# jonathandw743/black_hole_ray_marching

Measured on AMD Instinct MI355X. Metric: Mpix/s at 4096×2048, 512 RK steps; max |Δpixel| vs WGSL ref, higher is better.
Workload: dtype f32

## Files before the change

### black_hole_ray_marching_amd/__init__.py

```python
from ._abi import (BH_BLOOM_AUTO, BH_BLOOM_LITERAL, BH_FATE_BLACKOUT, BH_FATE_CAP, BH_FATE_ESCAPE, BH_FATE_SURFACE, BH_LAYOUT_ROWMAJOR,
                   BH_LAYOUT_TILES, BH_LAYOUT_TILES_RGB, BH_LAYOUT_TILES_RGBM, BH_LAYOUT_TILES_RGBM14, BH_UNPACK_RGBM14, BH_ORDER_STATES, BH_BLOOM_SETS, BH_MAX_FRAMES, BH_MATH_EXACT, BH_MATH_FAST, BH_OUT_BGRA8_SRGB, BH_OUT_RGBA16F,
                   BH_OUT_RGBA32F, BH_SCENE_DEFAULT, BH_SCENE_DISC, BH_SCENE_MARKERS, BH_SCHED_FLAG_STATIC_ORDER, BH_SCHED_FLAG_ISSUE_ORDER, BH_SCHED_FLAG_LATENCY, BH_SCHED_PAIR, BH_SCHED_PERSISTENT, BH_SCHED_TILE,
                   BH_LENS_BLACKOUT, BH_LENS_SURFACE, BYTES_PER_PIXEL,
                   BhError, load)
from .scene import (MAX_ITERATIONS, Camera, CameraController, CameraUniform, FrameBatch, Partition, Presenter, Scene, Sky, Uniforms, bloom_check, bloom_plan_failures, clock_mhz, lens_shade_host, load_sky, sky_mips_host,
                    partition_map, refine_cover_host, refine_mask_host, shard_tile_count, shutter_resolve_host, srgb_encode_table, ss_resolve_host, tiles_unpack_rgbm_partition,
                    synthetic_sky, tile_bytes, tiles_unpack, tiles_unpack_rgb, tiles_unpack_rgbm)
from . import raymap

__version__ = "0.5.0"
```

### black_hole_ray_marching_amd/_abi.py

```python
from __future__ import annotations

import ctypes as C
import os
from pathlib import Path

LIB_PATH = Path(os.environ.get("BH_LIB", Path(__file__).resolve().parent / "libbh_render.so"))

BH_OK = 0
BH_ERR_INVALID_ARG = -1
BH_ERR_UNSUPPORTED = -2
BH_ERR_HIP = -3
BH_ERR_NO_DEVICE = -4
BH_ERR_OUT_OF_MEMORY = -5
BH_ERR_INTERNAL = -6

BH_OUT_RGBA32F, BH_OUT_RGBA16F, BH_OUT_BGRA8_SRGB = 0, 1, 2
BH_BLOOM_AUTO, BH_BLOOM_LITERAL = 0, 1
BH_MATH_EXACT, BH_MATH_FAST = 0, 1
BH_SCENE_DISC, BH_SCENE_MARKERS = 1, 2
BH_SCENE_DEFAULT = 3
BH_LAYOUT_ROWMAJOR, BH_LAYOUT_TILES, BH_LAYOUT_TILES_RGB, BH_LAYOUT_TILES_RGBM, BH_LAYOUT_TILES_RGBM14 = 0, 1, 2, 3, 4
BH_UNPACK_RGBM14 = 0x100
BH_ORDER_STATES = 32
BH_BLOOM_SETS = 4
# ... 147 lines not shown
    "bh_tiles_unpack_rgb_rows": (C.c_int, [C.c_void_p, C.c_void_p, C.c_uint32, C.c_uint32, C.c_uint32,
                                           C.c_uint64, C.c_uint32, C.c_uint32, C.c_void_p]),
    "bh_tiles_unpack_rgbm": (C.c_int, [C.c_void_p, C.c_void_p, C.c_void_p, C.c_uint32, C.c_uint32, C.c_uint32,
                                       C.c_uint64, C.c_uint32, C.c_uint32, C.c_void_p]),
    "bh_tile_bytes": (C.c_int64, [C.c_uint32, C.c_uint32]),
    "bh_partition_create": (C.c_int, [C.c_uint32, C.c_uint32, C.c_uint32, C.POINTER(C.c_uint32), C.c_int,
                                      C.POINTER(C.c_void_p)]),
    "bh_partition_destroy": (C.c_int, [C.c_void_p]),
    "bh_partition_tile_count": (C.c_int64, [C.c_void_p, C.c_uint32]),
    "bh_partition_map": (C.c_int, [C.c_uint32, C.c_uint32, C.c_uint32, C.POINTER(C.c_uint32), C.c_void_p,
                                   C.c_void_p]),
    "bh_tiles_unpack_rgbm_partition": (C.c_int, [C.c_void_p, C.c_void_p, C.c_void_p, C.c_void_p, C.c_uint64,
                                                 C.c_uint32, C.c_uint32, C.c_void_p]),
    "bh_srgb_encode_table": (C.c_int, [C.c_void_p]),
    "bh_div_magic_misses": (C.c_int64, [C.c_uint32, C.c_uint32, C.POINTER(C.c_uint32)]),
    "bh_controller_update": (C.c_int, [C.POINTER(bh_controller), C.POINTER(bh_camera), C.c_float, C.c_int,
                                       C.POINTER(C.c_int)]),
    "bh_bloom": (C.c_int, [C.c_void_p, C.c_void_p, C.c_void_p, C.c_uint32, C.c_uint32, C.c_uint32, C.c_uint32,
                           C.c_void_p, C.c_void_p]),
    "bh_bloom_check": (C.c_int, [C.c_uint32, C.c_uint32, C.c_uint32, C.c_uint32, C.POINTER(C.c_uint64), C.c_char_p,
                                 C.c_size_t]),
    "bh_presenter_create": (C.c_int, [C.c_void_p, C.POINTER(bh_presenter_desc), C.POINTER(C.c_void_p)]),
    "bh_presenter_destroy": (C.c_int, [C.c_void_p]),
    "bh_present_frames": (C.c_int, [C.c_void_p, C.c_uint32, C.POINTER(bh_camera_uniform), C.POINTER(bh_uniforms),
                                    C.POINTER(C.c_void_p), C.c_void_p]),
    "bh_present": (C.c_int, [C.c_void_p, C.POINTER(bh_camera_uniform), C.POINTER(bh_uniforms), C.c_void_p, C.c_void_p]),
    "bh_bloom_plan_failures": (C.c_int64, [C.c_char_p, C.c_size_t]),
    "bh_selftest_crmath": (C.c_int, [C.c_int, C.c_uint64, C.c_uint64, C.POINTER(C.c_uint64), C.c_void_p, C.c_int]),
    "bh_set_clock_probe": (C.c_int, [C.c_void_p, C.c_void_p, C.c_uint32]),
    "bh_graph_release": (C.c_int, [C.c_void_p]),
# ... 43 lines not shown
```

### black_hole_ray_marching_amd/csrc/bh_common.hpp

```cpp
#pragma once
#include <hip/hip_runtime.h>
#include <stddef.h>
#include <stdint.h>

#include <string>

#include "../../include/bh_render.h"

namespace bh {

template <uint32_t V>
struct Const { static constexpr uint32_t value = V; };
template <class F>
__attribute__((visibility("hidden"))) inline int with_format(uint32_t format, F&& f) {
    switch (format) {
        case BH_OUT_RGBA32F: return f(Const<BH_OUT_RGBA32F>{});
        case BH_OUT_RGBA16F: return f(Const<BH_OUT_RGBA16F>{});
        default: return f(Const<BH_OUT_BGRA8_SRGB>{});
    }
}

constexpr uint32_t BH_INLINE_FRAMES = 32;
static_assert(BH_INLINE_FRAMES <= BH_MAX_FRAMES, "inline frames");

struct FrameArgs {
    float pos[3];
    float c0[3], c1[3], c2[3];
    float cps[3];
    void* out_col;
    void* out_blackout;
    uint16_t* dbg_n_rk;
    uint8_t* dbg_fate;
    uint16_t* dbg_steps;
};

struct MarchArgs {
    float pos[3];
    float c0[3], c1[3], c2[3];
    float rs, dtm, max_dist, dp;
    uint32_t blackout_eh;
    uint32_t skip_sdf;
    float far_r2;
    uint32_t ss_log2;
    uint32_t ss_out_width;
    uint32_t lens;
    uint32_t width, height, max_iters, scene_flags;
    uint32_t format, layout;
    uint32_t shard_index, shard_count;
    uint32_t tiles_x, tiles_y;
// ... 11 lines not shown
    const float* srgb_lut;
    const float* srgb_enc;
    uint32_t sky_w, sky_h;
    void* out_col;
    void* out_blackout;
    uint16_t* dbg_n_rk;
    uint8_t* dbg_fate;
    uint16_t* dbg_steps;
    uint32_t n_frames;
    uint32_t nf_magic;
    const FrameArgs* frame_table;
    unsigned long long* clk;
    uint32_t clk_mask;
    uint32_t tx_magic;
    FrameArgs frames[BH_INLINE_FRAMES];
};
inline uint32_t div_magic(uint32_t d, uint32_t n_max) {
    if (d < 2u) return 0u;
    const uint64_t m = (1ull << 32) / d + 1u, e = m * d - (1ull << 32);
    return (uint64_t)n_max * e < (1ull << 32) ? (uint32_t)m : 0u;
}
static_assert(sizeof(MarchArgs) + 8 <= 4096, "MarchArgs must fit the kernel argument segment");
static_assert(offsetof(MarchArgs, far_r2) == 72 && offsetof(MarchArgs, ss_log2) == 76 &&
                  offsetof(MarchArgs, ss_out_width) == 80 && offsetof(MarchArgs, lens) == 84 &&
                  offsetof(MarchArgs, width) == 88,
              "MarchArgs: the supersampling words must stay inside the former reserved_[3]");
static_assert(offsetof(MarchArgs, order) == 144 && offsetof(MarchArgs, sky) == 200 && offsetof(MarchArgs, out_col) == 232 &&
                  offsetof(MarchArgs, n_frames) == 272 && offsetof(MarchArgs, frames) == 304 &&
                  sizeof(FrameArgs) == 104 && sizeof(MarchArgs) == 304 + BH_INLINE_FRAMES * sizeof(FrameArgs),
              "MarchArgs: kernel argument layout changed");

struct RefineArgs {
    uint32_t* list;
    uint32_t* ctr;
    const uint8_t* tile_cost;
    uint8_t* mask;
    uint32_t* refined;
    uint32_t width, height;
    uint32_t tiles_x, tiles_y;
    uint32_t n_frames;
    uint32_t capacity;
    uint32_t n_heads;
    float thr;
};

struct LensShadeArgs {
    const bh_lens_px* lens;
    const uint32_t* sky;
    const float* srgb_lut;
    const float* srgb_enc;
    void* out_col;
    void* out_blackout;
    uint32_t width, height;
    uint32_t sky_w, sky_h;
};

struct LensMipArgs : LensShadeArgs {
    const void* chain;
    uint32_t n_levels;
// ... 115 lines not shown
```

### black_hole_ray_marching_amd/csrc/bh_host.cpp

```cpp
#include <hip/hip_runtime.h>

#include <algorithm>
#include <cmath>
#include <cstdlib>
#include <cstring>
#include <limits>
#include <new>
#include <string>
#include <vector>

#include "bh_host.hpp"
#include "bh_srgb.hpp"
#include "bh_lens.hpp"
#include "bh_refine.hpp"
#include "bh_shutter.hpp"
#include "bh_ss.hpp"

namespace {
thread_local std::string g_last_error;
}
static void free_frame_table(bh_ctx::FrameTable& t);

void srgb_lut(float lut[256]) {
    for (int i = 0; i < 256; ++i) {
// ... 240 lines not shown
    if (d->schedule & BH_SCHED_FLAG_ISSUE_ORDER) return true;
    if (d->schedule & BH_SCHED_FLAG_LATENCY) return false;
    const uint64_t tiles = (uint64_t)n_tiles * n_frames;
    return tiles * 512ull >= 384ull * (cus ? cus : 256u) * d->max_iters;
}

static void free_frame_table(bh_ctx::FrameTable& t) {
    for (uint32_t k = 0; k < bh_ctx::FRAME_RING; ++k) {
        if (t.done[k]) { (void)hipEventSynchronize(t.done[k]); (void)hipEventDestroy(t.done[k]); }
        if (t.host[k]) (void)hipHostFree(t.host[k]);
    }
    if (t.dev) (void)hipFree(t.dev);
    t = bh_ctx::FrameTable{};
}

static int stage_frame_table(bh_ctx* c, hipStream_t s, const bh::FrameArgs* frames, uint32_t n,
                             const bh::FrameArgs** dev) {
    if (stream_capturing(s)) {
        g_last_error = "bh_render_frames: more than 32 frames per call cannot be captured into a graph";
        return BH_ERR_UNSUPPORTED;
    }
    bh_ctx::FrameTable* t = nullptr;
    for (auto& x : c->frame_tables)
        if (x.stream == (void*)s) t = &x;
    if (!t) {
        bh_ctx::FrameTable n_t;
        n_t.stream = (void*)s;
        const size_t bytes = sizeof(bh::FrameArgs) * BH_MAX_FRAMES;
        hipError_t he = hipMalloc(&n_t.dev, bytes);
        for (uint32_t k = 0; he == hipSuccess && k < bh_ctx::FRAME_RING; ++k) {
            he = hipHostMalloc(&n_t.host[k], bytes, hipHostMallocDefault);
            if (he == hipSuccess) he = hipEventCreateWithFlags(&n_t.done[k], hipEventDisableTiming);
        }
        if (he != hipSuccess) {
            free_frame_table(n_t);
            return alloc_fail(he, "frame table");
        }
        c->frame_tables.push_back(n_t);
        t = &c->frame_tables.back();
    }
    *dev = t->dev;
    if (t->last.size() == n && std::memcmp(t->last.data(), frames, sizeof(bh::FrameArgs) * n) == 0) return BH_OK;
    const uint32_t k = t->next;
    t->next = (k + 1u) % bh_ctx::FRAME_RING;
    hipError_t he = hipEventSynchronize(t->done[k]);
    if (he == hipSuccess) {
        std::memcpy(t->host[k], frames, sizeof(bh::FrameArgs) * n);
        he = hipMemcpyAsync(t->dev, t->host[k], sizeof(bh::FrameArgs) * n, hipMemcpyHostToDevice, s);
    }
    if (he == hipSuccess) he = hipEventRecord(t->done[k], s);
    if (he != hipSuccess) {
        t->last.clear();
        return hip_fail(he, "frame table upload");
    }
    t->last.assign(frames, frames + n);
    return BH_OK;
}

static int order_state(bh_ctx* c, const bh_render_desc* d, uint64_t nt, hipStream_t s, bool capturing,
                       bh_ctx::OrderState** out, bool from_map = false) {
    const uint64_t pser = d->partition ? d->partition->serial : 0u;
    for (auto& o : c->orders)
        if (o.matches(d, pser, nt, s, from_map)) {
            o.last_use = ++c->order_clock;
            if (capturing) {
                if (!o.valid) {
                    g_last_error = "bh_render: this (geometry, shard, stream) must be rendered once outside graph capture";
                    return BH_ERR_UNSUPPORTED;
                }
                o.captured = true;
// ... 37 lines not shown
}

static void frame_args(const bh_camera_uniform* cam, float rs, const bh_render_desc* d, bh::FrameArgs* F) {
    for (int k = 0; k < 3; ++k) {
        F->pos[k] = cam->pos[k];
        F->c0[k] = cam->world_tri[0][k];
        F->c1[k] = cam->world_tri[1][k];
        F->c2[k] = cam->world_tri[2][k];
    }
    const float x = F->pos[0], y = F->pos[1], z = F->pos[2];
    const float len = std::sqrt((x * x + y * y) + z * z);
    const float n[3] = {x / len, y / len, z / len};
    for (int k = 0; k < 3; ++k) F->cps[k] = (-n[k] * 1.5f) * rs;
    F->out_col = d->out_col; F->out_blackout = d->out_blackout;
    F->dbg_n_rk = d->dbg_n_rk; F->dbg_fate = d->dbg_fate; F->dbg_steps = d->dbg_steps;
}

static uint64_t frame_cost_key(const bh_camera_uniform* cam, const bh_uniforms* U, const bh_render_desc* d,
                               const float* ray_map = nullptr, const bh_ray_pose* poses = nullptr, uint32_t n_poses = 0u,
                               const float* origin_map = nullptr) {
    uint64_t h = 1469598103934665603ull;
    auto mix = [&](const void* p, size_t n) {
        const unsigned char* b = static_cast<const unsigned char*>(p);
        for (size_t i = 0; i < n; ++i) h = (h ^ b[i]) * 1099511628211ull;
    };
    mix(cam->pos, sizeof(float) * 3);
    for (int k = 0; k < 3; ++k) mix(cam->world_tri[k], sizeof(float) * 3);
    for (int k = 0; k < 3; ++k) mix(cam->screen_tri[k], sizeof(float) * 3);
    mix(&U->rs, 4); mix(&U->delta_time_mult, 4); mix(&U->blackout_eh, 4); mix(&U->max_dist, 4);
    mix(&U->distortion_power, 4);
// ... 47 lines not shown
        const char* why = e->layout != BH_LAYOUT_ROWMAJOR      ? "a row-major output (BH_LAYOUT_ROWMAJOR)"
                          : e->shard_count != 1u               ? "the whole frame (shard_count 1)"
                          : e->partition                       ? "no partition"
                          : (e->schedule & 0xFFu) != BH_SCHED_TILE ? "the tile schedule (BH_SCHED_TILE)"
                          : (e->dbg_n_rk || e->dbg_fate || e->dbg_steps) ? "no dbg_* outputs (they are per ray, not per pixel)"
                                                               : nullptr;
        if (why) return why;
    }
    return nullptr;
}

struct Launch {
    bh_render_desc d;
    bh::MarchArgs a;
    std::vector<bh::FrameArgs> table;
    uint64_t n_tiles = 0;
    uint32_t shutter_log2 = 0;
    const float* ray_map = nullptr;
    const bh_ray_pose* poses = nullptr;
    const float* origin_map = nullptr;
};

static int check_launch(const bh_ctx* c, uint32_t n_frames, const bh_camera_uniform* cams, const bh_uniforms* U,
                        const bh_render_desc* descs, uint32_t ss, Launch* L) {
    if (!c || !cams || !U || !descs || n_frames == 0 || n_frames > BH_MAX_FRAMES) return bad_arg(__func__, __LINE__);
    const bh_render_desc* const d0 = &descs[0];
    L->d = *d0;
    if (ss > 1u) { L->d.width *= ss; L->d.height *= ss; }
    const bh_render_desc* d = &L->d;
    if (!d->out_col) return bad_arg(__func__, __LINE__);
// ... 54 lines not shown
    a.order_block = (uint32_t)((L->n_tiles + a.tiles_y - 1u) / a.tiles_y);
    a.order_centre = bh_tile_row(&cams[0], d->height);
    a.sky = c->sky; a.srgb_lut = c->lut; a.srgb_enc = c->enc; a.sky_w = c->sky_w; a.sky_h = c->sky_h;
    a.kfac = (a.dp * a.rs) * -1.5f;
    a.rw2 = 1.0f / (2.0f * (float)a.width);
    a.rh2 = 1.0f / (2.0f * (float)a.height);
    a.n_frames = n_frames;
    const uint64_t slots = L->n_tiles * n_frames;
    a.nf_magic = slots - 1u <= 0xFFFFFFFFull ? bh::div_magic(n_frames, (uint32_t)(slots - 1u)) : 0u;
    a.tx_magic = a.shard_count == 1u && a.n_tiles != 0u ? bh::div_magic(a.tiles_x, a.n_tiles - 1u) : 0u;
    a.clk = c->clk;
    a.clk_mask = c->clk_mask;
    if (n_frames > bh::BH_INLINE_FRAMES) L->table.resize(n_frames);
    bh::FrameArgs* fa = L->table.empty() ? a.frames : L->table.data();
    for (uint32_t i = 0; i < n_frames; ++i) frame_args(&cams[i], a.rs, &descs[i], &fa[i]);
    const bh::FrameArgs& F = fa[0];
    for (int k = 0; k < 3; ++k) {
        a.pos[k] = F.pos[k]; a.c0[k] = F.c0[k]; a.c1[k] = F.c1[k]; a.c2[k] = F.c2[k]; a.cps[k] = F.cps[k];
    }
    a.out_col = F.out_col; a.out_blackout = F.out_blackout;
    a.dbg_n_rk = F.dbg_n_rk; a.dbg_fate = F.dbg_fate; a.dbg_steps = F.dbg_steps;
}

static int stage_frames(bh_ctx* c, hipStream_t s, Launch* L) {
    if (L->table.empty()) return BH_OK;
    return stage_frame_table(c, s, L->table.data(), L->a.n_frames, &L->a.frame_table);
}

static int learned_order(bh_ctx* c, Launch* L, const bh_camera_uniform* cam0, const bh_uniforms* U, hipStream_t s,
                         bh_ctx::OrderState** out) {
    const bh_render_desc* d = &L->d;
    bh::MarchArgs& a = L->a;
    *out = nullptr;
    if ((d->schedule & 0xFFu) != BH_SCHED_TILE || (d->schedule & BH_SCHED_FLAG_STATIC_ORDER)) return BH_OK;
    bh_ctx::OrderState* os = nullptr;
    int st = order_state(c, d, L->n_tiles, s, stream_capturing(s), &os, L->ray_map != nullptr);
    if (st != BH_OK) return st;
    if (!os->valid) {
        hipError_t he = hipMemsetAsync(os->counters, 0, bh::ORDER_WORDS * sizeof(uint32_t), s);
        if (he == hipSuccess) he = hipMemsetAsync(os->tile_cost, 0, L->n_tiles, s);
        if (he != hipSuccess) return hip_fail(he, "temporal order reset");
// ... 540 lines not shown
```

### black_hole_ray_marching_amd/csrc/bh_host.hpp

```cpp
#pragma once
#include <hip/hip_runtime.h>

#include <array>
#include <cstring>
#include <memory>
#include <string>
#include <vector>

#include "bh_common.hpp"
#include "bh_srgb.hpp"

#define BH_HIDDEN __attribute__((visibility("hidden")))
#define BH_INTERNAL extern "C" BH_HIDDEN

struct bh_ctx {
    int device = 0;
    uint32_t* sky = nullptr;
    float* lut = nullptr;
    float* enc = nullptr;
    uint8_t* enc_b = nullptr;
    uint32_t* enc_e = nullptr;
    uint32_t* counters = nullptr;
    uint32_t sky_w = 0, sky_h = 0;
    uint32_t grid_exact = 0, grid_fast = 0;
// ... 24 lines not shown
        void free_buffers() {
            (void)hipFree(tile_cost); (void)hipFree(order); (void)hipFree(counters);
            (void)hipFree(refine_list); (void)hipFree(refine_ctr); (void)hipFree(refine_mask);
        }
    };
    std::vector<OrderState> orders;
    uint64_t order_clock = 0;
    static constexpr uint32_t FRAME_RING = 4;
    struct FrameTable {
        void* stream = nullptr;
        bh::FrameArgs* dev = nullptr;
        bh::FrameArgs* host[FRAME_RING] = {};
        hipEvent_t done[FRAME_RING] = {};
        uint32_t next = 0;
        std::vector<bh::FrameArgs> last;
    };
    std::vector<FrameTable> frame_tables;
    struct SepPlan {
        std::array<uint32_t, 6> key{};
        uint32_t* dev = nullptr;
        int ext = 0;
        uint32_t nc = 0, nr = 0;
        size_t rec = 0;
        size_t stc = 0;
        uint32_t stw = 0;
        uint32_t* strips = nullptr;
        std::shared_ptr<std::vector<uint32_t>> host;
    };
    struct BloomScratch {
        uint64_t key = 0;
// ... 137 lines not shown
```

### black_hole_ray_marching_amd/csrc/bh_march_ray.hpp

```cpp
#pragma once
#include "bh_march_step.hpp"

namespace bh {
namespace BH_NS {

constexpr uint32_t PRIO_ITERS = 48;

constexpr uint32_t WG_WAVES = 1u;

struct Hist { v3 ro, rd; float tr; uint32_t outside; };

__device__ __forceinline__ bool same_bits(float x, float y) { return __float_as_uint(x) == __float_as_uint(y); }
__device__ __forceinline__ bool same_state(const RayState& st, const Hist& h) {
    return same_bits(st.ro.x, h.ro.x) & same_bits(st.ro.y, h.ro.y) & same_bits(st.ro.z, h.ro.z) &
           same_bits(st.rd.x, h.rd.x) & same_bits(st.rd.y, h.rd.y) & same_bits(st.rd.z, h.rd.z) &
           same_bits(st.travelled, h.tr) & (st.outside == h.outside);
}

struct HistLds { float4 a[2][2][64]; };
__device__ __forceinline__ uint32_t state_hash(const RayState& st) {
    return (__float_as_uint(st.ro.x) ^ __float_as_uint(st.ro.y) ^ __float_as_uint(st.ro.z) ^
            __float_as_uint(st.rd.x) ^ __float_as_uint(st.rd.y) ^ __float_as_uint(st.rd.z) ^
            __float_as_uint(st.travelled)) + st.outside * 0x9E3779B9u;
}
// ... 35 lines not shown
                    const float4 r0 = H.a[p][0][lane], r1 = H.a[p][1][lane];
                    st.ro = mk(r0.x, r0.y, r0.z); st.rd = mk(r1.x, r1.y, r1.z); st.travelled = r0.w;
                }
                st.n_rk = a.max_iters;
                return BH_FATE_CAP;
            }
        }
        h2 = h1;
    }
    for (;;) {
        const uint32_t fate = march_step_tail<SF>(a, f, st);
        if (fate != 0xFFu) { steps = st.n_rk; return fate; }
    }
}

template <uint32_t SF, bool SHUT = false>
__device__ __forceinline__ void march_ray(const MarchArgs& a, const Frame& f, RayState& st, uint32_t& fate,
                                          uint32_t& steps, uint32_t lane) {
    RayState sb = st;
    bool alive = true;
    constexpr uint32_t TRIP_PAIRS = 3;
    static_assert(PRIO_ITERS % (2u * TRIP_PAIRS) == 0u, "whole trips");
    for (uint32_t it = 0; it < PRIO_ITERS && __builtin_amdgcn_ballot_w64(alive) != 0ull; it += 2u * TRIP_PAIRS) {
#pragma unroll
        for (uint32_t j = 0; j < TRIP_PAIRS; ++j) {
            if (alive) {
                if (march_step_io<SF, true>(a, f, st, sb, fate, it + 2u * j)) {
                    alive = false;
                    if (fate_before_rk(fate)) sb.n_rk = 0u;
                }
            }
            if (alive) {
                if (march_step_io<SF, true>(a, f, sb, st, fate, it + 2u * j + 1u)) {
                    alive = false;
                    if (fate_before_rk(fate)) st.n_rk = 0u;
                }
            }
        }
// ... 12 lines not shown
```

### black_hole_ray_marching_amd/csrc/bh_march_step.hpp

```cpp
#pragma once
#include "bh_march_ops.hpp"

namespace bh {
namespace BH_NS {


struct Frame {
    v3 ro0;
    v3 cps;
    float k;
};
__device__ __forceinline__ Frame make_frame(const MarchArgs& a) {
    Frame f;
    f.ro0 = mk(a.pos[0], a.pos[1], a.pos[2]);
    f.cps = mk(a.cps[0], a.cps[1], a.cps[2]);
    f.k = a.kfac;
    return f;
}

__device__ __forceinline__ v3 pixel_ray(const MarchArgs& a, uint32_t px, uint32_t py) {
#if BH_FAST
    const float l0 = ((float)px + 0.5f) / (2.0f * (float)a.width);
    const float l2 = ((float)py + 0.5f) / (2.0f * (float)a.height);
#else
// ... 352 lines not shown
    G.bad |= !(G.amin >= crm::ACC_N_MIN);
    if constexpr (!CO) G.bad |= !(fabsf(s) <= 0x1p30f);
    const float ntr = travelled + dt;
    out.s = s;
    out.outside = CO ? 1u : (not_out ? in.outside : 1u);
    out.ro = unpk(padd(ro, dro));
    out.rd = unpk(padd(rd, drd));
    out.travelled = ntr;
    out.n_rk = n_rk + 1u;
    const bool escape = ntr > a.max_dist;
    fate = escape ? (uint32_t)BH_FATE_ESCAPE : (uint32_t)BH_FATE_CAP;
    return escape | (n_rk + 1u >= a.max_iters);
}
#endif

template <uint32_t SF = SF_DYN, bool UNI = false, bool TINY = false>
__device__ __forceinline__ bool march_step_io(const MarchArgs& a, const Frame& f, const RayState& in, RayState& out,
                                              uint32_t& fate, uint32_t it = 0u) {
#if BH_FAST
    FOps X;
    return step_bf<true, FOps, SF, UNI>(a, f, in, out, X, fate, it);
#else
    XOps<true> X;
#ifdef BH_DIAG_SLOW
    if ((threadIdx.x & 63u) == (uint32_t)__builtin_ctzll(__builtin_amdgcn_ballot_w64(true)))
        atomicAdd(&g_diag_all_wave_steps, 1u);
#endif
    bool done = step_bf<true, XOps<true>, SF, UNI, TINY>(a, f, in, out, X, fate, it);
#ifdef BH_DIAG_SLOW
    const uint64_t badm = __builtin_amdgcn_ballot_w64(X.bad);
// ... 75 lines not shown
```

### black_hole_ray_marching_amd/csrc/bh_march_tile.hpp

```cpp
#pragma once
#include "bh_march_ray.hpp"
#include "bh_march_resolve.hpp"
#include "bh_march_shade.hpp"
#include "bh_refine.hpp"

namespace bh {
namespace BH_NS {


#define BH_CONST_AS __attribute__((address_space(4)))
template <class T>
__device__ __forceinline__ const BH_CONST_AS T* const_as(const T* p) { return (const BH_CONST_AS T*)p; }
__device__ __forceinline__ const BH_CONST_AS FrameArgs* frame_args_of(const MarchArgs& A, uint32_t fi) {
    return (A.frame_table ? const_as(A.frame_table) : const_as(&A.frames[0])) + fi;
}
struct FrameCamera { float pos[3], c0[3], c1[3], c2[3], cps[3]; };
__device__ __forceinline__ FrameCamera load_camera(const BH_CONST_AS FrameArgs* F) {
    FrameCamera c;
    for (int k = 0; k < 3; ++k) {
        c.pos[k] = F->pos[k]; c.c0[k] = F->c0[k]; c.c1[k] = F->c1[k]; c.c2[k] = F->c2[k]; c.cps[k] = F->cps[k];
    }
    return c;
}
__device__ __forceinline__ void select_camera(MarchArgs& a, const FrameCamera& c) {
    for (int k = 0; k < 3; ++k) {
        a.pos[k] = c.pos[k]; a.c0[k] = c.c0[k]; a.c1[k] = c.c1[k]; a.c2[k] = c.c2[k]; a.cps[k] = c.cps[k];
    }
}
__device__ __forceinline__ void select_outputs(MarchArgs& a, const BH_CONST_AS FrameArgs* F) {
    a.out_col = F->out_col; a.out_blackout = F->out_blackout;
    a.dbg_n_rk = F->dbg_n_rk; a.dbg_fate = F->dbg_fate; a.dbg_steps = F->dbg_steps;
}

struct SlotHead {
    uint32_t fi, t, tx, ty;
    FrameCamera cam;
    bool ok;
};
template <bool ITEM>
__device__ __forceinline__ SlotHead slot_head(const MarchArgs& A, uint32_t slot, uint32_t item_tx = 0u, uint32_t item_ty = 0u) {
    SlotHead h{};
    const uint32_t nf = A.n_frames;
    uint32_t fi = 0, j = slot;
    if constexpr (ITEM) {
        fi = slot;
    } else if (nf > 1u) {
        j = A.nf_magic ? __umulhi(slot, A.nf_magic) : slot / nf;
        fi = slot - j * nf;
    }
    h.fi = fi;
    h.cam = load_camera(frame_args_of(A, fi));
    if constexpr (ITEM) {
        h.tx = item_tx;
        h.ty = item_ty;
    } else {
        const uint32_t t = A.order ? const_as(A.order)[j] : centre_out(j, A.n_tiles, A.order_block, A.order_centre);
        h.t = t;
        if (t >= A.n_tiles) return h;
        if (A.tile_list) {
            const uint32_t v = const_as(A.tile_list)[t];
            h.tx = v & 0xFFFFu;
            h.ty = v >> 16;
        } else if (A.shard_count == 1u && A.tx_magic) {
            h.ty = __umulhi(t, A.tx_magic);
            h.tx = t - h.ty * A.tiles_x;
        } else {
            shard_tile_coords(t, A.tiles_x, A.shard_index, A.shard_count, &h.tx, &h.ty);
        }
    }
    h.ok = true;
    return h;
}

constexpr uint32_t F_SS = 1u, F_ITEM = 2u, F_LENS = 4u, F_SHUT = 8u, F_RAYS = 16u, F_POSE = 32u, F_ORG = 64u;
struct ShutterLane { uint32_t px, py; bool valid, ok; };
struct OrgRay { v3 d, ro0; };
__device__ __forceinline__ OrgRay org_load(const MarchArgs& a, const float* dirs, const float* orgs, uint32_t px,
                                           uint32_t py, bool valid) {
    OrgRay g;
    g.d = mk(0.0f, 0.0f, 1.0f);
    g.ro0 = mk(a.pos[0], a.pos[1], a.pos[2]);
    if (valid) {
        const size_t i = ((size_t)py * a.width + px) * 3u;
        const float* p = dirs + i;
        const float* q = orgs + i;
        const v3 m = mk(p[0], p[1], p[2]);
        const v3 o = mk(q[0], q[1], q[2]);
        const v3 r = mk(a.c0[0], a.c0[1], a.c0[2]), u = mk(a.c1[0], a.c1[1], a.c1[2]), fw = mk(a.c2[0], a.c2[1], a.c2[2]);
        g.d = add(add(smul(m.x, r), smul(m.y, u)), smul(m.z, fw));
// ... 56 lines not shown
            const float* p = dirs + ((size_t)py * a.width + px) * 3u;
            d = mk(p[0], p[1], p[2]);
            if constexpr (POSE)
                d = add(add(smul(d.x, mk(a.c0[0], a.c0[1], a.c0[2])), smul(d.y, mk(a.c1[0], a.c1[1], a.c1[2]))),
                        smul(d.z, mk(a.c2[0], a.c2[1], a.c2[2])));
        }
        st.rd = normalize_x(d);
    } else
#endif
    st.rd = pixel_ray(a, valid ? px : 0u, valid ? py : 0u);
    st.s = ray_s(f, st.rd);
    st.travelled = 0.0f;
    st.n_rk = 0;
    st.outside = 0u;
    uint32_t fate = 0xFFu, steps = 0;
    if (valid) {
        if constexpr (SF != SF_DYN) {
            const bool out = ORG ? __builtin_amdgcn_ballot_w64(!((dot(f.ro0, f.ro0) > 1.01f) & (fabsf(st.s) <= 0x1p30f))) == 0ull
                                 : (dot(f.ro0, f.ro0) > 1.01f) && (__builtin_amdgcn_ballot_w64(!(fabsf(st.s) <= 0x1p30f)) == 0ull);
            if (__builtin_amdgcn_readfirstlane((int)out)) march_ray<SF | SF_CAM_OUT, SHUT>(a, f, st, fate, steps, lane);
            else march_ray<SF, SHUT>(a, f, st, fate, steps, lane);
        } else {
            march_ray<SF, SHUT>(a, f, st, fate, steps, lane);
        }
    }
    if constexpr (SHUT) {
        shutter_stage(a, lut, lane, valid, fate, st, steps);
        *sl = ShutterLane{px, py, valid, true};
    } else
    if constexpr (SS) {
        uint32_t fo = fi;
        asm volatile("" : "+s"(fo));
        select_outputs(a, frame_args_of(A, fo));
        v3 sc, sb;
        ss_samples(a, lut, lane, valid, fate, st, steps, sc, sb);
        ss_resolve_store<FMT>(a, lut, lane, px, py, valid, sc, sb);
    } else
    if (valid) {
// ... 13 lines not shown
    if (a.tile_cost) {
        const uint32_t m = min(wave_max_u32(steps) >> 1, 255u);
        if (lane == 0u) {
            a.tile_cost[t] = (uint8_t)m;
            const uint32_t b = cost_bucket(m);
            if (b < ORDER_BUCKETS - 1u)
                __hip_atomic_fetch_add(&a.order_tot[b], 1u, __ATOMIC_RELAXED, __HIP_MEMORY_SCOPE_AGENT);
        }
    }
}
template <uint32_t FMT, uint32_t SF, uint32_t FORM>
__device__ __forceinline__ void march_slot(const MarchArgs& A, uint32_t slot, const float* lut,
                                           uint32_t lane, uint32_t item_tx = 0u, uint32_t item_ty = 0u,
                                           ShutterLane* sl = nullptr, const float* dirs = nullptr,
                                           const float* orgs = nullptr) {
    const SlotHead h = slot_head<(FORM & F_ITEM) != 0u>(A, slot, item_tx, item_ty);
    if (!h.ok) return;
    march_slot_body<FMT, SF, FORM>(A, h, lut, lane, sl, dirs, orgs);
}

struct ClockStart { uint32_t t, r; };
__device__ __forceinline__ ClockStart clock_start() {
    return {(uint32_t)__builtin_amdgcn_s_memtime(), (uint32_t)__builtin_amdgcn_s_memrealtime()};
}
__device__ __forceinline__ void clock_end(unsigned long long* acc, const ClockStart& c0) {
    const uint32_t t = (uint32_t)__builtin_amdgcn_s_memtime() - c0.t;
    const uint32_t r = (uint32_t)__builtin_amdgcn_s_memrealtime() - c0.r;
    const uint32_t x = __builtin_amdgcn_s_getreg((3 << 11) | (0 << 6) | 20) & 7u;
    const bool sane = (uint64_t)t >= 5ull * r && (uint64_t)t <= 40ull * r;
    if ((threadIdx.x & 63u) == 0u && sane) {
        unsigned long long* p = acc + 16u * x;
// ... 4 lines not shown
}

template <uint32_t FMT, uint32_t SF, uint32_t FORM>
__device__ __forceinline__ void march_tile_wave(const MarchArgs& A, float* lut, const float* dirs = nullptr,
                                                const float* orgs = nullptr) {
    static_assert(WG_WAVES == 1u, "the table copy is one wave's: 64 lanes x 16 bytes per table");
    static_assert(!(FORM & (F_ITEM | F_SHUT)), "work items and shutter waves have kernels of their own");
    constexpr bool LENS = FORM & F_LENS;
    asm volatile("" ::"s"(A.srgb_lut), "s"(A.n_tiles), "s"(A.n_frames), "s"(A.nf_magic), "s"(A.frame_table),
                 "s"(A.order), "s"(A.tile_list), "s"(A.shard_count), "s"(A.tx_magic), "s"(A.tiles_x), "s"(A.clk),
                 "s"(A.clk_mask), "s"(A.width), "s"(A.height), "s"(A.rw2), "s"(A.rh2));
    SrgbRows<FMT> rows;
    if constexpr (!LENS) rows = srgb_fetch<FMT>(A);
    const uint32_t slot = __builtin_amdgcn_readfirstlane(blockIdx.x * WG_WAVES + (threadIdx.x >> 6));
    if (slot >= A.n_tiles * A.n_frames) return;
    const SlotHead h = slot_head<false>(A, slot);
    if constexpr (!LENS) {
        srgb_store<FMT>(rows, lut);
        __syncthreads();
    }
    const bool probe = A.clk && ((slot + (slot >> 8)) & A.clk_mask) == 0u;
    ClockStart c0{0u, 0u};
    if (probe) c0 = clock_start();
    if (h.ok) march_slot_body<FMT, SF, FORM>(A, h, lut, threadIdx.x & 63u, nullptr, dirs, orgs);
    if (probe) clock_end(A.clk, c0);
}

template <uint32_t FMT, uint32_t SF>
__global__ void __launch_bounds__(64 * WG_WAVES) march_tile_kernel(MarchArgs A) {
    __shared__ __attribute__((aligned(16))) float lut[lds_tables<FMT>()];
    march_tile_wave<FMT, SF, 0u>(A, lut);
// ... 160 lines not shown
```

### black_hole_ray_marching_amd/scene.py

```python
from __future__ import annotations

import ctypes as C
from dataclasses import dataclass, field

import numpy as np

from . import _abi
from ._abi import (BH_LAYOUT_ROWMAJOR, BH_LAYOUT_TILES, BH_LAYOUT_TILES_RGB, BH_LAYOUT_TILES_RGBM, BH_LAYOUT_TILES_RGBM14, BH_UNPACK_RGBM14, BH_MATH_EXACT, BH_MATH_FAST, BH_OUT_RGBA16F,
                   BH_OUT_RGBA32F, BH_OUT_BGRA8_SRGB, BH_SCENE_DEFAULT, BYTES_PER_PIXEL, BhError, check, load)

MAX_ITERATIONS = 1000


@dataclass
class Camera:
    pos: tuple = (0.0, 0.0, -20.0)
    dir: tuple = (0.0, 0.0, 1.0)
    up: tuple = (0.0, 1.0, 0.0)
    aspect: float = 1.0
    fovy: float = float(np.float32(np.pi) * np.float32(0.5))
    znear: float = 0.1
    zfar: float = 100.0

    @classmethod
# ... 110 lines not shown
    out = np.empty((height, width, 4), dtype=np.uint8)
    check(load().bh_synthetic_sky(out.ctypes.data, width, height, seed), "bh_synthetic_sky")
    return out


def load_sky(path) -> np.ndarray:
    from PIL import Image
    with Image.open(path) as im:
        return np.ascontiguousarray(np.asarray(im.convert("RGBA"), dtype=np.uint8))


def srgb_encode_table() -> np.ndarray:
    out = np.empty(257, np.float32)
    check(load().bh_srgb_encode_table(out.ctypes.data), "bh_srgb_encode_table")
    return out


def shard_tile_count(width: int, height: int, shard_index: int, shard_count: int) -> int:
    n = load().bh_shard_tile_count(width, height, shard_index, shard_count)
    if n < 0:
        raise BhError(int(n), "bh_shard_tile_count")
    return int(n)


def bloom_check(width: int, height: int, levels: int = 3, schedule: int = 0) -> list[tuple]:
    lib = load()
    n = C.c_uint64()
    buf = C.create_string_buffer(1 << 16)
    check(lib.bh_bloom_check(width, height, levels, schedule, C.byref(n), buf, len(buf)), "bh_bloom_check")
    out = []
# ... 734 lines not shown
```

### include/bh_render.h

```cpp
#ifndef BH_RENDER_H
#define BH_RENDER_H

#include <stddef.h>
#include <stdint.h>

#ifdef __cplusplus
extern "C" {
#endif

#define BH_ABI_VERSION 8

#define BH_ORDER_STATES 32
#define BH_BLOOM_SETS 4

typedef enum {
    BH_OK = 0,
    BH_ERR_INVALID_ARG = -1,
    BH_ERR_UNSUPPORTED = -2,
    BH_ERR_HIP = -3,
    BH_ERR_NO_DEVICE = -4,
    BH_ERR_OUT_OF_MEMORY = -5,
    BH_ERR_INTERNAL = -6
} bh_status;

// ... 257 lines not shown
                        bh_partition** out);
int bh_partition_destroy(bh_partition* partition);
int64_t bh_partition_tile_count(const bh_partition* partition, uint32_t shard_index);
int bh_partition_map(uint32_t width, uint32_t height, uint32_t shard_count, const uint32_t* weights, uint32_t* owner_out,
                     uint32_t* index_out);
int bh_tiles_unpack_rgbm_partition(const void* packed, void* out_col, void* out_blackout, const bh_partition* partition,
                                   uint64_t shard_stride_tiles, uint32_t format, uint32_t rows_in_flight,
                                   void* hip_stream);

int64_t bh_tile_bytes(uint32_t layout, uint32_t format);

int bh_srgb_encode_table(float* out257);

int64_t bh_div_magic_misses(uint32_t d, uint32_t n_max, uint32_t* magic);

int bh_selftest_crmath(int op, uint64_t base, uint64_t count, uint64_t* out_mismatches,
                       uint32_t* out_examples, int device);

int bh_set_clock_probe(bh_ctx* ctx, uint64_t* acc, uint32_t stride);

#ifdef __cplusplus
}
#endif

#endif
```

Baseline: 16720.

## Peel first RK step using host-precomputed per-frame step size and radius terms

All rays in a frame start at the camera position, so the first step's SDF distance, step size and 1/r^5 divisor are identical across pixels. The host now computes these once per frame and passes them in the kernel arguments or frame table, and the tile kernel runs a specialised first RK4 step that skips the SDF evaluation and one divide. The main march loop then resumes at iteration 1. This adds kernel-argument bytes, a validity fallback through a wave ballot, and extra code paths that could raise register pressure.

```diff
diff --git a/black_hole_ray_marching_amd/__init__.py b/black_hole_ray_marching_amd/__init__.py
--- a/black_hole_ray_marching_amd/__init__.py
+++ b/black_hole_ray_marching_amd/__init__.py
@@ -3,7 +3,7 @@
                    BH_OUT_RGBA32F, BH_SCENE_DEFAULT, BH_SCENE_DISC, BH_SCENE_MARKERS, BH_SCHED_FLAG_STATIC_ORDER, BH_SCHED_FLAG_ISSUE_ORDER, BH_SCHED_FLAG_LATENCY, BH_SCHED_PAIR, BH_SCHED_PERSISTENT, BH_SCHED_TILE,
                    BH_LENS_BLACKOUT, BH_LENS_SURFACE, BYTES_PER_PIXEL,
                    BhError, load)
-from .scene import (MAX_ITERATIONS, Camera, CameraController, CameraUniform, FrameBatch, Partition, Presenter, Scene, Sky, Uniforms, bloom_check, bloom_plan_failures, clock_mhz, lens_shade_host, load_sky, sky_mips_host,
+from .scene import (MAX_ITERATIONS, Camera, CameraController, CameraUniform, FrameBatch, Partition, Presenter, Scene, Sky, Uniforms, bloom_check, bloom_plan_failures, clock_mhz, first_step_host, lens_shade_host, load_sky, sky_mips_host,
                     partition_map, refine_cover_host, refine_mask_host, shard_tile_count, shutter_resolve_host, srgb_encode_table, ss_resolve_host, tiles_unpack_rgbm_partition,
                     synthetic_sky, tile_bytes, tiles_unpack, tiles_unpack_rgb, tiles_unpack_rgbm)
 from . import raymap
diff --git a/black_hole_ray_marching_amd/_abi.py b/black_hole_ray_marching_amd/_abi.py
--- a/black_hole_ray_marching_amd/_abi.py
+++ b/black_hole_ray_marching_amd/_abi.py
@@ -185,6 +185,8 @@
                                                  C.c_uint32, C.c_uint32, C.c_void_p]),
     "bh_srgb_encode_table": (C.c_int, [C.c_void_p]),
     "bh_div_magic_misses": (C.c_int64, [C.c_uint32, C.c_uint32, C.POINTER(C.c_uint32)]),
+    "bh_first_step_host": (C.c_int, [C.POINTER(bh_camera_uniform), C.POINTER(bh_uniforms), C.c_uint32, C.c_uint32,
+                                     C.POINTER(C.c_float), C.POINTER(C.c_float), C.POINTER(C.c_float)]),
     "bh_controller_update": (C.c_int, [C.POINTER(bh_controller), C.POINTER(bh_camera), C.c_float, C.c_int,
                                        C.POINTER(C.c_int)]),
     "bh_bloom": (C.c_int, [C.c_void_p, C.c_void_p, C.c_void_p, C.c_uint32, C.c_uint32, C.c_uint32, C.c_uint32,
diff --git a/black_hole_ray_marching_amd/csrc/bh_common.hpp b/black_hole_ray_marching_amd/csrc/bh_common.hpp
--- a/black_hole_ray_marching_amd/csrc/bh_common.hpp
+++ b/black_hole_ray_marching_amd/csrc/bh_common.hpp
@@ -33,6 +33,8 @@
     uint8_t* dbg_fate;
     uint16_t* dbg_steps;
 };
+
+struct FirstStep { float dt0, Q0, rq0; };
 
 struct MarchArgs {
     float pos[3];
@@ -74,20 +76,22 @@
     uint32_t clk_mask;
     uint32_t tx_magic;
     FrameArgs frames[BH_INLINE_FRAMES];
+    FirstStep first[BH_INLINE_FRAMES];
 };
 inline uint32_t div_magic(uint32_t d, uint32_t n_max) {
     if (d < 2u) return 0u;
     const uint64_t m = (1ull << 32) / d + 1u, e = m * d - (1ull << 32);
     return (uint64_t)n_max * e < (1ull << 32) ? (uint32_t)m : 0u;
 }
-static_assert(sizeof(MarchArgs) + 8 <= 4096, "MarchArgs must fit the kernel argument segment");
+static_assert(sizeof(MarchArgs) + 16 <= 4096, "MarchArgs must fit the kernel argument segment");
 static_assert(offsetof(MarchArgs, far_r2) == 72 && offsetof(MarchArgs, ss_log2) == 76 &&
                   offsetof(MarchArgs, ss_out_width) == 80 && offsetof(MarchArgs, lens) == 84 &&
                   offsetof(MarchArgs, width) == 88,
               "MarchArgs: the supersampling words must stay inside the former reserved_[3]");
 static_assert(offsetof(MarchArgs, order) == 144 && offsetof(MarchArgs, sky) == 200 && offsetof(MarchArgs, out_col) == 232 &&
                   offsetof(MarchArgs, n_frames) == 272 && offsetof(MarchArgs, frames) == 304 &&
-                  sizeof(FrameArgs) == 104 && sizeof(MarchArgs) == 304 + BH_INLINE_FRAMES * sizeof(FrameArgs),
+                  sizeof(FrameArgs) == 104 && offsetof(MarchArgs, first) == 304 + BH_INLINE_FRAMES * sizeof(FrameArgs) &&
+                  sizeof(FirstStep) == 12 && sizeof(MarchArgs) == 304 + BH_INLINE_FRAMES * (sizeof(FrameArgs) + sizeof(FirstStep)),
               "MarchArgs: kernel argument layout changed");
 
 struct RefineArgs {
@@ -103,6 +107,7 @@
     uint32_t n_heads;
     float thr;
 };
+static_assert(sizeof(MarchArgs) + sizeof(RefineArgs) <= 4096, "march_refine_kernel's arguments must fit the kernel argument segment");
 
 struct LensShadeArgs {
     const bh_lens_px* lens;
diff --git a/black_hole_ray_marching_amd/csrc/bh_host.cpp b/black_hole_ray_marching_amd/csrc/bh_host.cpp
--- a/black_hole_ray_marching_amd/csrc/bh_host.cpp
+++ b/black_hole_ray_marching_amd/csrc/bh_host.cpp
@@ -278,8 +278,8 @@
     t = bh_ctx::FrameTable{};
 }
 
-static int stage_frame_table(bh_ctx* c, hipStream_t s, const bh::FrameArgs* frames, uint32_t n,
-                             const bh::FrameArgs** dev) {
+static int stage_frame_table(bh_ctx* c, hipStream_t s, const bh::FrameArgs* frames, const bh::FirstStep* first,
+                             uint32_t n, const bh::FrameArgs** dev) {
     if (stream_capturing(s)) {
         g_last_error = "bh_render_frames: more than 32 frames per call cannot be captured into a graph";
         return BH_ERR_UNSUPPORTED;
@@ -290,7 +290,7 @@
     if (!t) {
         bh_ctx::FrameTable n_t;
         n_t.stream = (void*)s;
-        const size_t bytes = sizeof(bh::FrameArgs) * BH_MAX_FRAMES;
+        const size_t bytes = (sizeof(bh::FrameArgs) + sizeof(bh::FirstStep)) * BH_MAX_FRAMES;
         hipError_t he = hipMalloc(&n_t.dev, bytes);
         for (uint32_t k = 0; he == hipSuccess && k < bh_ctx::FRAME_RING; ++k) {
             he = hipHostMalloc(&n_t.host[k], bytes, hipHostMallocDefault);
@@ -304,13 +304,17 @@
         t = &c->frame_tables.back();
     }
     *dev = t->dev;
-    if (t->last.size() == n && std::memcmp(t->last.data(), frames, sizeof(bh::FrameArgs) * n) == 0) return BH_OK;
+    const size_t fb = sizeof(bh::FrameArgs) * n, rb = sizeof(bh::FirstStep) * n;
+    if (t->last.size() == n && std::memcmp(t->last.data(), frames, fb) == 0 &&
+        std::memcmp(t->last_first.data(), first, rb) == 0)
+        return BH_OK;
     const uint32_t k = t->next;
     t->next = (k + 1u) % bh_ctx::FRAME_RING;
     hipError_t he = hipEventSynchronize(t->done[k]);
     if (he == hipSuccess) {
-        std::memcpy(t->host[k], frames, sizeof(bh::FrameArgs) * n);
-        he = hipMemcpyAsync(t->dev, t->host[k], sizeof(bh::FrameArgs) * n, hipMemcpyHostToDevice, s);
+        std::memcpy(t->host[k], frames, fb);
+        std::memcpy(reinterpret_cast<unsigned char*>(t->host[k]) + fb, first, rb);
+        he = hipMemcpyAsync(t->dev, t->host[k], fb + rb, hipMemcpyHostToDevice, s);
     }
     if (he == hipSuccess) he = hipEventRecord(t->done[k], s);
     if (he != hipSuccess) {
@@ -318,6 +322,7 @@
         return hip_fail(he, "frame table upload");
     }
     t->last.assign(frames, frames + n);
+    t->last_first.assign(first, first + n);
     return BH_OK;
 }
 
@@ -385,6 +390,60 @@
     for (int k = 0; k < 3; ++k) F->cps[k] = (-n[k] * 1.5f) * rs;
     F->out_col = d->out_col; F->out_blackout = d->out_blackout;
     F->dbg_n_rk = d->dbg_n_rk; F->dbg_fate = d->dbg_fate; F->dbg_steps = d->dbg_steps;
+}
+
+static bool first_step_disabled() {
+    static const bool off = std::getenv("BH_NO_FIRST_STEP") != nullptr;
+    return off;
+}
+
+static bool first_step_record(const float pos[3], const float cps[3], float rs, float dtm, float max_dist,
+                              uint32_t scene_flags, uint32_t max_iters, bh::FirstStep* out) {
+    *out = bh::FirstStep{0.0f, 0.0f, 0.0f};
+    const float x = pos[0], y = pos[1], z = pos[2];
+    const float in[8] = {x, y, z, cps[0], cps[1], cps[2], rs, dtm};
+    for (float v : in)
+        if (!std::isfinite(v)) return false;
+    if (!(dtm > 0.0f) || !(rs > 0.0f) || !(max_iters >= 2u)) return false;
+    const float r2 = (x * x + y * y) + z * z;
+    if (!(r2 > 1.01f && r2 <= 0x1p24f)) return false;
+    const float r0 = std::sqrt(r2);
+    const float dtr = dtm * r0;
+    const float rho = std::sqrt(x * x + z * z);
+    const float disc = std::fmax(std::fmax(rho - 6.0f * rs, -(rho - 3.0f * rs)), std::fabs(y - 0.0f) - 0.02f);
+    const float xx = x * x, yy = y * y;
+    const float dz = -10.0f - z, zz = dz * dz;
+    const float ty = 10.0f - std::fabs(y), tx = 10.0f - std::fabs(x);
+    const float qy = (xx + ty * ty) + zz, qx = (tx * tx + yy) + zz;
+    const float m = std::sqrt(std::fmin(qy, qx)) - 0.5f;
+    float ds;
+    if (!(scene_flags & BH_SCENE_MARKERS)) ds = (scene_flags & BH_SCENE_DISC) ? disc : INFINITY;
+    else ds = (scene_flags & BH_SCENE_DISC) ? std::fmin(disc, m) : m;
+    if (!(ds >= 0.001f)) return false;
+    const float dx = cps[0] - x, dy = cps[1] - y, dzp = cps[2] - z;
+    const float dps = std::sqrt((dx * dx + dy * dy) + dzp * dzp) - 0.075f;
+    const float dist = std::fmin(ds, dps);
+    const float dt0 = std::fmin(dist * 0.9f, dtr);
+    if (!(dt0 >= 0x1p-25f && dt0 <= 0x1p13f) || !(dt0 <= max_dist)) return false;
+    const float Q0 = (r2 * r2) * r0;
+    const float rq0 = 1.0f / Q0;
+    if (!(Q0 >= 0x1p-40f && Q0 <= 0x1p60f)) return false;
+    *out = bh::FirstStep{dt0, Q0, rq0};
+    return true;
+}
+
+int bh_first_step_host(const bh_camera_uniform* cam, const bh_uniforms* U, uint32_t scene_flags, uint32_t max_iters,
+                       float* dt0, float* Q0, float* rq0) {
+    if (!cam || !U) return 0;
+    bh::FrameArgs F;
+    bh_render_desc d{};
+    frame_args(cam, U->rs, &d, &F);
+    bh::FirstStep fs;
+    const bool ok = first_step_record(F.pos, F.cps, U->rs, U->delta_time_mult, U->max_dist, scene_flags, max_iters, &fs);
+    if (dt0) *dt0 = fs.dt0;
+    if (Q0) *Q0 = fs.Q0;
+    if (rq0) *rq0 = fs.rq0;
+    return ok ? 1 : 0;
 }
 
 static uint64_t frame_cost_key(const bh_camera_uniform* cam, const bh_uniforms* U, const bh_render_desc* d,
@@ -462,6 +521,7 @@
     bh_render_desc d;
     bh::MarchArgs a;
     std::vector<bh::FrameArgs> table;
+    std::vector<bh::FirstStep> first_table;
     uint64_t n_tiles = 0;
     uint32_t shutter_log2 = 0;
     const float* ray_map = nullptr;
@@ -546,6 +606,11 @@
     if (n_frames > bh::BH_INLINE_FRAMES) L->table.resize(n_frames);
     bh::FrameArgs* fa = L->table.empty() ? a.frames : L->table.data();
     for (uint32_t i = 0; i < n_frames; ++i) frame_args(&cams[i], a.rs, &descs[i], &fa[i]);
+    if (!L->table.empty()) L->first_table.assign(n_frames, bh::FirstStep{0.0f, 0.0f, 0.0f});
+    bh::FirstStep* fs = L->table.empty() ? a.first : L->first_table.data();
+    if (d->math == BH_MATH_EXACT && (d->schedule & 0xFFu) == BH_SCHED_TILE && !first_step_disabled())
+        for (uint32_t i = 0; i < n_frames; ++i)
+            (void)first_step_record(fa[i].pos, fa[i].cps, a.rs, a.dtm, a.max_dist, a.scene_flags, a.max_iters, &fs[i]);
     const bh::FrameArgs& F = fa[0];
     for (int k = 0; k < 3; ++k) {
         a.pos[k] = F.pos[k]; a.c0[k] = F.c0[k]; a.c1[k] = F.c1[k]; a.c2[k] = F.c2[k]; a.cps[k] = F.cps[k];
@@ -556,7 +621,7 @@
 
 static int stage_frames(bh_ctx* c, hipStream_t s, Launch* L) {
     if (L->table.empty()) return BH_OK;
-    return stage_frame_table(c, s, L->table.data(), L->a.n_frames, &L->a.frame_table);
+    return stage_frame_table(c, s, L->table.data(), L->first_table.data(), L->a.n_frames, &L->a.frame_table);
 }
 
 static int learned_order(bh_ctx* c, Launch* L, const bh_camera_uniform* cam0, const bh_uniforms* U, hipStream_t s,
diff --git a/black_hole_ray_marching_amd/csrc/bh_host.hpp b/black_hole_ray_marching_amd/csrc/bh_host.hpp
--- a/black_hole_ray_marching_amd/csrc/bh_host.hpp
+++ b/black_hole_ray_marching_amd/csrc/bh_host.hpp
@@ -62,6 +62,7 @@
         hipEvent_t done[FRAME_RING] = {};
         uint32_t next = 0;
         std::vector<bh::FrameArgs> last;
+        std::vector<bh::FirstStep> last_first;
     };
     std::vector<FrameTable> frame_tables;
     struct SepPlan {
diff --git a/black_hole_ray_marching_amd/csrc/bh_march_ray.hpp b/black_hole_ray_marching_amd/csrc/bh_march_ray.hpp
--- a/black_hole_ray_marching_amd/csrc/bh_march_ray.hpp
+++ b/black_hole_ray_marching_amd/csrc/bh_march_ray.hpp
@@ -73,14 +73,17 @@
     }
 }
 
-template <uint32_t SF, bool SHUT = false>
+template <uint32_t SF, bool SHUT = false, bool PEEL = false>
 __device__ __forceinline__ void march_ray(const MarchArgs& a, const Frame& f, RayState& st, uint32_t& fate,
-                                          uint32_t& steps, uint32_t lane) {
+                                          uint32_t& steps, uint32_t lane, [[maybe_unused]] const RayState* prev = nullptr,
+                                          [[maybe_unused]] uint32_t it0 = 0u) {
     RayState sb = st;
+    if constexpr (PEEL) sb = *prev;
+    const uint32_t first = PEEL ? it0 : 0u;
     bool alive = true;
     constexpr uint32_t TRIP_PAIRS = 3;
     static_assert(PRIO_ITERS % (2u * TRIP_PAIRS) == 0u, "whole trips");
-    for (uint32_t it = 0; it < PRIO_ITERS && __builtin_amdgcn_ballot_w64(alive) != 0ull; it += 2u * TRIP_PAIRS) {
+    for (uint32_t it = first; it < PRIO_ITERS + first && __builtin_amdgcn_ballot_w64(alive) != 0ull; it += 2u * TRIP_PAIRS) {
 #pragma unroll
         for (uint32_t j = 0; j < TRIP_PAIRS; ++j) {
             if (alive) {
diff --git a/black_hole_ray_marching_amd/csrc/bh_march_step.hpp b/black_hole_ray_marching_amd/csrc/bh_march_step.hpp
--- a/black_hole_ray_marching_amd/csrc/bh_march_step.hpp
+++ b/black_hole_ray_marching_amd/csrc/bh_march_step.hpp
@@ -390,6 +390,40 @@
 }
 #endif
 
+#if !BH_FAST
+__device__ __forceinline__ bool step_first(const RayState& in, RayState& out, const FirstStep& fs) {
+    XOps<true> X;
+    const v3 ro = in.ro, rd = in.rd;
+    const float s = in.s, dt = fs.dt0;
+    const float nx = s * ro.x, ny = s * ro.y, nz = s * ro.z;
+    X.kmin = crm::kmin3(crm::key(nx), crm::key(ny), crm::key(nz));
+    const crm::Rcp R{fs.Q0, fs.rq0};
+    const v3 ro_k1 = smul(dt, rd);
+    const v3 rd_k1 = smul(dt, mk(crm::div_core(nx, R), crm::div_core(ny, R), crm::div_core(nz, R)));
+    const v3 ro_k2 = smul(dt, X.rd_half(rd, rd_k1));
+    const v3 rd_k2 = smul(dt, X.template accel<2>(X.ro_half(ro, ro_k1), s));
+    const v3 ro_k3 = smul(dt, X.rd_half(rd, rd_k2));
+    const v3 rd_k3 = smul(dt, X.template accel<3>(X.ro_half(ro, ro_k2), s));
+    const v3 ro_k4 = smul(dt, add(rd, rd_k3));
+    const v3 rd_k4 = smul(dt, X.template accel<4>(add(ro, ro_k3), s));
+    const v3 sro = add(X.add2(X.add2(ro_k1, ro_k2), ro_k3), ro_k4);
+    const v3 srd = add(X.add2(X.add2(rd_k1, rd_k2), rd_k3), rd_k4);
+    const v3 dro = X.template div6<0>(sro);
+    const v3 drd = X.template div6<1>(srd);
+    X.bad |= X.kmin < crm::KEY_ACC_MIN;
+    X.bad |= !(X.amin >= crm::ACC_N_MIN);
+    X.bad |= !(X.amin6 >= crm::DIV_N_MIN);
+    X.bad |= !(fabsf(s) <= 0x1p30f);
+    out.ro = add(ro, dro);
+    out.rd = add(rd, drd);
+    out.travelled = in.travelled + dt;
+    out.s = s;
+    out.n_rk = in.n_rk + 1u;
+    out.outside = 1u;
+    return X.bad;
+}
+#endif
+
 template <uint32_t SF = SF_DYN, bool UNI = false, bool TINY = false>
 __device__ __forceinline__ bool march_step_io(const MarchArgs& a, const Frame& f, const RayState& in, RayState& out,
                                               uint32_t& fate, uint32_t it = 0u) {
diff --git a/black_hole_ray_marching_amd/csrc/bh_march_tile.hpp b/black_hole_ray_marching_amd/csrc/bh_march_tile.hpp
--- a/black_hole_ray_marching_amd/csrc/bh_march_tile.hpp
+++ b/black_hole_ray_marching_amd/csrc/bh_march_tile.hpp
@@ -35,9 +35,15 @@
 struct SlotHead {
     uint32_t fi, t, tx, ty;
     FrameCamera cam;
+    FirstStep fs;
     bool ok;
 };
-template <bool ITEM>
+__device__ __forceinline__ FirstStep load_first_step(const MarchArgs& A, uint32_t fi) {
+    const BH_CONST_AS FirstStep* p = A.frame_table ? (const BH_CONST_AS FirstStep*)(const_as(A.frame_table) + A.n_frames)
+                                                   : const_as(&A.first[0]);
+    return {p[fi].dt0, p[fi].Q0, p[fi].rq0};
+}
+template <bool ITEM, bool FS = false>
 __device__ __forceinline__ SlotHead slot_head(const MarchArgs& A, uint32_t slot, uint32_t item_tx = 0u, uint32_t item_ty = 0u) {
     SlotHead h{};
     const uint32_t nf = A.n_frames;
@@ -50,6 +56,7 @@
     }
     h.fi = fi;
     h.cam = load_camera(frame_args_of(A, fi));
+    if constexpr (FS) h.fs = load_first_step(A, fi);
     if constexpr (ITEM) {
         h.tx = item_tx;
         h.ty = item_ty;
@@ -73,6 +80,7 @@
 }
 
 constexpr uint32_t F_SS = 1u, F_ITEM = 2u, F_LENS = 4u, F_SHUT = 8u, F_RAYS = 16u, F_POSE = 32u, F_ORG = 64u;
+constexpr bool form_first_step(uint32_t form) { return !BH_FAST && !(form & F_ORG); }
 struct ShutterLane { uint32_t px, py; bool valid, ok; };
 struct OrgRay { v3 d, ro0; };
 __device__ __forceinline__ OrgRay org_load(const MarchArgs& a, const float* dirs, const float* orgs, uint32_t px,
@@ -159,14 +167,34 @@
     st.n_rk = 0;
     st.outside = 0u;
     uint32_t fate = 0xFFu, steps = 0;
+    constexpr bool PEEL = form_first_step(FORM);
     if (valid) {
+        [[maybe_unused]] RayState s0 = st;
+        [[maybe_unused]] uint32_t it0 = 0u;
+#if !BH_FAST
+        if constexpr (PEEL) {
+            if (h.fs.Q0 != 0.0f) {
+                RayState s1;
+                const bool bad = step_first(st, s1, h.fs);
+                if (__builtin_amdgcn_ballot_w64(bad) == 0ull) {
+                    st = s1;
+                    it0 = 1u;
+                }
+            }
+        }
+#endif
         if constexpr (SF != SF_DYN) {
             const bool out = ORG ? __builtin_amdgcn_ballot_w64(!((dot(f.ro0, f.ro0) > 1.01f) & (fabsf(st.s) <= 0x1p30f))) == 0ull
-                                 : (dot(f.ro0, f.ro0) > 1.01f) && (__builtin_amdgcn_ballot_w64(!(fabsf(st.s) <= 0x1p30f)) == 0ull);
-            if (__builtin_amdgcn_readfirstlane((int)out)) march_ray<SF | SF_CAM_OUT, SHUT>(a, f, st, fate, steps, lane);
-            else march_ray<SF, SHUT>(a, f, st, fate, steps, lane);
+                                 : (PEEL && it0 != 0u) ||
+                                   ((dot(f.ro0, f.ro0) > 1.01f) && (__builtin_amdgcn_ballot_w64(!(fabsf(st.s) <= 0x1p30f)) == 0ull));
+            if (__builtin_amdgcn_readfirstlane((int)out)) {
+                march_ray<SF | SF_CAM_OUT, SHUT, PEEL>(a, f, st, fate, steps, lane, &s0, it0);
+            } else {
+                if constexpr (PEEL) st = s0;
+                march_ray<SF, SHUT>(a, f, st, fate, steps, lane);
+            }
         } else {
-            march_ray<SF, SHUT>(a, f, st, fate, steps, lane);
+            march_ray<SF, SHUT, PEEL>(a, f, st, fate, steps, lane, &s0, it0);
         }
     }
     if constexpr (SHUT) {
@@ -210,7 +238,7 @@
                                            uint32_t lane, uint32_t item_tx = 0u, uint32_t item_ty = 0u,
                                            ShutterLane* sl = nullptr, const float* dirs = nullptr,
                                            const float* orgs = nullptr) {
-    const SlotHead h = slot_head<(FORM & F_ITEM) != 0u>(A, slot, item_tx, item_ty);
+    const SlotHead h = slot_head<(FORM & F_ITEM) != 0u, form_first_step(FORM)>(A, slot, item_tx, item_ty);
     if (!h.ok) return;
     march_slot_body<FMT, SF, FORM>(A, h, lut, lane, sl, dirs, orgs);
 }
@@ -245,7 +273,7 @@
     if constexpr (!LENS) rows = srgb_fetch<FMT>(A);
     const uint32_t slot = __builtin_amdgcn_readfirstlane(blockIdx.x * WG_WAVES + (threadIdx.x >> 6));
     if (slot >= A.n_tiles * A.n_frames) return;
-    const SlotHead h = slot_head<false>(A, slot);
+    const SlotHead h = slot_head<false, form_first_step(FORM)>(A, slot);
     if constexpr (!LENS) {
         srgb_store<FMT>(rows, lut);
         __syncthreads();
diff --git a/black_hole_ray_marching_amd/scene.py b/black_hole_ray_marching_amd/scene.py
--- a/black_hole_ray_marching_amd/scene.py
+++ b/black_hole_ray_marching_amd/scene.py
@@ -148,6 +148,14 @@
     out = np.empty(257, np.float32)
     check(load().bh_srgb_encode_table(out.ctypes.data), "bh_srgb_encode_table")
     return out
+
+
+def first_step_host(camera_uniform: "CameraUniform", uniforms: "Uniforms", scene_flags: int = BH_SCENE_DEFAULT,
+                    max_iters: int = 512) -> tuple[bool, np.float32, np.float32, np.float32]:
+    dt0, q0, rq0 = C.c_float(), C.c_float(), C.c_float()
+    ok = load().bh_first_step_host(C.byref(camera_uniform.c), C.byref(uniforms.to_c()), scene_flags, max_iters,
+                                   C.byref(dt0), C.byref(q0), C.byref(rq0))
+    return bool(ok), np.float32(dt0.value), np.float32(q0.value), np.float32(rq0.value)
 
 
 def shard_tile_count(width: int, height: int, shard_index: int, shard_count: int) -> int:
diff --git a/include/bh_render.h b/include/bh_render.h
--- a/include/bh_render.h
+++ b/include/bh_render.h
@@ -295,6 +295,9 @@
 
 int64_t bh_div_magic_misses(uint32_t d, uint32_t n_max, uint32_t* magic);
 
+int bh_first_step_host(const bh_camera_uniform* camera, const bh_uniforms* uniforms, uint32_t scene_flags,
+                       uint32_t max_iters, float* dt0, float* Q0, float* rq0);
+
 int bh_selftest_crmath(int op, uint64_t base, uint64_t count, uint64_t* out_mismatches,
                        uint32_t* out_examples, int device);
 
```

New measurement: 17080 (median of 6 runs). 1.02x the previous value.
